# antgroup/ant-ray

Measured on NVIDIA H100. Metric: resnet50_ddp_train_images_per_sec, higher is better.
Workload: dtype bf16

## Files before the change

### ant-ray_b200/csrc/inst_norm.cu

```cuda
#include <algorithm>

#include "norm_kernels.cuh"
#include "norm_launch.h"

namespace b200c {
namespace bn {

static int ceil_div(int a, int b) { return (a + b - 1) / b; }

static int last_pow2(unsigned n) {
  n |= (n >> 1);
  n |= (n >> 2);
  n |= (n >> 4);
  n |= (n >> 8);
  n |= (n >> 16);
  return std::max<int>(1, n - (n >> 1));
}

static void reduce_config(int reduction, int stride, dim3* block, dim3* grid) {
  int block_x = std::min(last_pow2(stride), kTileW);
  int block_y = std::min(last_pow2(ceil_div(reduction, kElemsPerThread)), kMaxBlock / block_x);
  if (block_x * block_y != kMaxBlock) block_x = std::min(last_pow2(stride), kMaxBlock / block_y);
  int grid_y = std::min(ceil_div(reduction, block_y * kElemsPerThread), kMaxHBlock);
  *block = dim3(block_x, block_y, 1);
  *grid = dim3(ceil_div(stride, block_x), grid_y < 8 ? 1 : grid_y, 1);
}

static_assert(kEwVec % kStatsVec == 0, "vec_ok covers the statistics kernel's vector width");
static bool vec_ok(int stride, const void* const* ptrs, int n) {
  if (stride % kEwVec) return false;
  for (int i = 0; i < n; i++)
    if (reinterpret_cast<uintptr_t>(ptrs[i]) % 16) return false;
  return true;
}

static void ew_config(int reduction, int stride, int vec, dim3* block, dim3* grid) {
  const int groups = stride / vec;
  const int bx = std::min(groups, kEwThreads);
  const int by = kEwThreads / bx;
  const int gx = ceil_div(groups, bx);
  const int gy = std::max(1, std::min(ceil_div(reduction, by), 4096 / gx));
  *block = dim3(bx, by, 1);
  *grid = dim3(gx, gy, 1);
}

constexpr int kSemaphores = kMaxChannels / kTileW;
constexpr size_t kSemaphoreBytes = (size_t)kSemaphores * 4;

size_t scratch_bytes(int stride) {
  return kSemaphoreBytes + (size_t)3 * stride * kMaxHBlock * 4 + (size_t)2 * stride * 4;
}

struct Scratch {
  int* semaphores;
  float* staging;
  float* sums;
};
static Scratch carve(void* scratch, int stride) {
  char* p = static_cast<char*>(scratch);
  Scratch s;
  s.semaphores = reinterpret_cast<int*>(p);
  s.staging = reinterpret_cast<float*>(p + kSemaphoreBytes);
  s.sums = s.staging + (size_t)3 * stride * kMaxHBlock;
  return s;
}

cudaError_t forward(const FwdArgs& a, cudaStream_t st) {
  Scratch s = carve(a.scratch, a.c);
  dim3 block, grid;
  reduce_config(a.m, a.c, &block, &grid);
  StatsOut o{a.save_mean, a.save_invstd, a.running_mean, a.running_var, a.num_batches_tracked, a.momentum,
             (float)((double)a.m / (double)(a.m - 1)), a.eps};
  const bf16* x = static_cast<const bf16*>(a.x);
  if (vec_ok(a.c, &a.x, 1)) {
    k_bn_stats<kStatsVec><<<grid, dim3(block.x / kStatsVec, block.y), 0, st>>>(x, o, s.staging, s.semaphores, a.m, a.c);
  } else {
    k_bn_stats<1><<<grid, block, 0, st>>>(x, o, s.staging, s.semaphores, a.m, a.c);
  }
  const void* ptrs[3] = {a.x, a.y, a.identity ? a.identity : a.x};
  const int vec = vec_ok(a.c, ptrs, 3) ? kEwVec : 1;
  ew_config(a.m, a.c, vec, &block, &grid);
  const bf16* id = static_cast<const bf16*>(a.identity);
  bf16* y = static_cast<bf16*>(a.y);
#define B200C_BN_TRANSFORM(V, R) k_bn_transform<V, R><<<grid, block, 0, st>>>(x, id, y, a.save_mean, a.save_invstd, a.weight, a.bias, a.m, a.c)
  if (vec == kEwVec) {
    if (id) B200C_BN_TRANSFORM(kEwVec, true); else B200C_BN_TRANSFORM(kEwVec, false);
  } else {
    if (id) B200C_BN_TRANSFORM(1, true); else B200C_BN_TRANSFORM(1, false);
  }
#undef B200C_BN_TRANSFORM
  return cudaGetLastError();
}

cudaError_t backward(const BwdArgs& a, cudaStream_t st) {
  Scratch s = carve(a.scratch, a.c);
  float* sum_dy = s.sums;
  float* sum_dy_xmu = s.sums + a.c;
  dim3 block, grid;
  reduce_config(a.m, a.c, &block, &grid);
  const bf16* x = static_cast<const bf16*>(a.x);
  const bf16* dy = static_cast<const bf16*>(a.dy);
  const bf16* y = static_cast<const bf16*>(a.y);
  bf16* masked = static_cast<bf16*>(a.dy_masked);
  k_bn_bwd_reduce<<<grid, block, 0, st>>>(x, dy, y, masked, a.save_mean, a.save_invstd, sum_dy, sum_dy_xmu, a.grad_weight,
                                          a.grad_bias, s.staging, s.semaphores, a.m, a.c);
  const void* ptrs[4] = {a.x, a.dy, a.y, a.dx};
  const void* mptrs[3] = {a.x, a.dy_masked, a.dx};
  const int vec = (masked ? vec_ok(a.c, mptrs, 3) : vec_ok(a.c, ptrs, 4)) ? kEwVec : 1;
  ew_config(a.m, a.c, vec, &block, &grid);
  const float norm_fct = (float)(1.0 / a.m);
  bf16* dx = static_cast<bf16*>(a.dx);
#define B200C_BN_ELEMT(V, M, G) \
  k_bn_bwd_elemt<V, M><<<grid, block, 0, st>>>(G, y, x, dx, a.save_mean, a.save_invstd, a.weight, sum_dy, sum_dy_xmu, norm_fct, a.m, a.c)
  if (vec == kEwVec) {
    if (masked) B200C_BN_ELEMT(kEwVec, true, masked); else B200C_BN_ELEMT(kEwVec, false, dy);
  } else {
    if (masked) B200C_BN_ELEMT(1, true, masked); else B200C_BN_ELEMT(1, false, dy);
  }
#undef B200C_BN_ELEMT
  return cudaGetLastError();
}

}
}
```

### ant-ray_b200/csrc/norm_kernels.cuh

```cuda
#pragma once
#include <cuda_bf16.h>
#include <cuda_runtime.h>
#include <stdint.h>

namespace b200c {
namespace bn {

constexpr int kMaxBlock = 512;
constexpr int kParallelLoads = 4;
constexpr int kElemsPerThread = 16;
constexpr int kTileW = 32;
constexpr int kMaxHBlock = 128;
constexpr int kStatsVec = 4;
constexpr int kEwThreads = 256;
constexpr int kEwVec = 8;

typedef __nv_bfloat16 bf16;

template <int V>
struct alignas(2 * V) BVec {
  bf16 v[V];
};


template <bool FUSE_NEW>
__device__ __forceinline__ void welford_merge_element(int& count, float& mean, float& m2n, const int& count_new,
                                                      const float& mean_new, const float& m2n_new) {
  float factor = float(1.0) / ::max(1, (count + count_new));
  float delta0 = mean - mean_new;
  const float c = count, c_new = count_new;
  mean = __fmul_rn(FUSE_NEW ? __fmaf_rn(mean_new, c_new, __fmul_rn(mean, c)) : __fmaf_rn(mean, c, __fmul_rn(mean_new, c_new)),
                   factor);
  m2n = __fadd_rn(m2n, __fmaf_rn(__fmul_rn(__fmul_rn(__fmul_rn(delta0, delta0), c_new), c), factor, m2n_new));
  count += count_new;
}

template <int V>
__device__ __forceinline__ void welford_merge_block_vertical(int (&count)[V], float (&mean)[V], float (&m2n)[V],
                                                             int* shmem_count, float* shmem_mean, float* shmem_m2n) {
  const int block_x = blockDim.x * V;
  auto address_base = threadIdx.x * V + threadIdx.y * block_x;
#pragma unroll
  for (int offset = blockDim.y / 2; offset > 0; offset >>= 1) {
    if (threadIdx.y < offset * 2) {
#pragma unroll
      for (int k = 0; k < V; k++) {
        shmem_mean[address_base + k] = mean[k];
        shmem_m2n[address_base + k] = m2n[k];
        shmem_count[address_base + k] = count[k];
      }
    }
    __syncthreads();
    if (threadIdx.y < offset && threadIdx.y + offset < blockDim.y) {
      auto address = address_base + offset * block_x;
#pragma unroll
      for (int k = 0; k < V; k++) {
        auto count_new = shmem_count[address + k];
        auto mean_new = shmem_mean[address + k];
        auto m2n_new = shmem_m2n[address + k];
        welford_merge_element<false>(count[k], mean[k], m2n[k], count_new, mean_new, m2n_new);
      }
    }
  }
}

__device__ __forceinline__ void merge_block_vertical_backward(float& sum_dy, float& sum_dy_xmu, float* shmem_sum_dy,
                                                              float* shmem_sum_dy_xmu) {
  auto address_base = threadIdx.x + threadIdx.y * blockDim.x;
#pragma unroll
  for (int offset = blockDim.y / 2; offset > 0; offset >>= 1) {
    if (threadIdx.y < offset * 2) {
      shmem_sum_dy[address_base] = sum_dy;
      shmem_sum_dy_xmu[address_base] = sum_dy_xmu;
    }
    __syncthreads();
    if (threadIdx.y < offset && threadIdx.y + offset < blockDim.y) {
      auto address = address_base + offset * blockDim.x;
      sum_dy += shmem_sum_dy[address];
      sum_dy_xmu += shmem_sum_dy_xmu[address];
    }
  }
}

struct StatsOut {
  float* save_mean;
  float* save_invstd;
  float* running_mean;
  float* running_var;
  long long* num_batches_tracked;
  float momentum, bessel, eps;
};

__device__ __forceinline__ void finish_stats(const StatsOut& o, int c, float mean_th, float m2_th, int count_th) {
  const float mean = mean_th;
  const float var = m2_th / count_th;
  const float momentum = o.momentum;
  const float unbiased_var = var * o.bessel;
  o.save_mean[c] = mean;
  o.running_mean[c] = __fmaf_rn(mean, momentum, __fmul_rn(1 - momentum, o.running_mean[c]));
  o.running_var[c] = __fmaf_rn(unbiased_var, momentum, __fmul_rn(1 - momentum, o.running_var[c]));
  o.save_invstd[c] = rsqrtf(var + o.eps);
}

template <int V>
__global__ void __launch_bounds__(kMaxBlock / V) k_bn_stats(const bf16* __restrict__ input, StatsOut o, volatile float* staging_data,
                                                            int* semaphores, const int reduction_size, const int stride) {
  constexpr int PARALLEL_LOADS = kParallelLoads;
  float x_mean[PARALLEL_LOADS][V];
  float m_2_n[PARALLEL_LOADS][V];
  int count[PARALLEL_LOADS];
#pragma unroll
  for (int i = 0; i < PARALLEL_LOADS; i++) {
#pragma unroll
    for (int k = 0; k < V; k++) {
      x_mean[i][k] = 0.f;
      m_2_n[i][k] = 0.f;
    }
    count[i] = 0;
  }
  if (o.num_batches_tracked && blockIdx.x == 0 && blockIdx.y == 0 && threadIdx.x == 0 && threadIdx.y == 0)
    *o.num_batches_tracked += 1;

  int inner_loop_stride = blockDim.y * gridDim.y;
  int m_offset = blockIdx.y * blockDim.y + threadIdx.y;
  int c_offset = (blockIdx.x * blockDim.x + threadIdx.x) * V;
  int loop_count = 1 + (reduction_size - 1) / (inner_loop_stride * PARALLEL_LOADS);
  const bool c_valid = c_offset < stride;

  for (int i = 0; i < loop_count; i++) {
    BVec<V> xv[PARALLEL_LOADS];
#pragma unroll
    for (int j = 0; j < PARALLEL_LOADS; j++) {
      const int m = m_offset + j * inner_loop_stride;
      if (c_valid && m < reduction_size) xv[j] = *reinterpret_cast<const BVec<V>*>(input + ((size_t)m * stride + c_offset));
    }
#pragma unroll
    for (int j = 0; j < PARALLEL_LOADS; j++) {
      float x_math[V];
      float x_count_inv;
      float is_valid;
      if (c_valid && m_offset < reduction_size) {
#pragma unroll
        for (int k = 0; k < V; k++) x_math[k] = __bfloat162float(xv[j].v[k]);
        count[j]++;
        x_count_inv = float(1) / count[j];
        is_valid = float(1);
      } else {
#pragma unroll
        for (int k = 0; k < V; k++) x_math[k] = float(0);
        x_count_inv = float(0);
        is_valid = float(0);
      }
      m_offset += inner_loop_stride;
#pragma unroll
      for (int k = 0; k < V; k++) {
        float delta0 = x_math[k] - x_mean[j][k];
        x_mean[j][k] = __fmaf_rn(delta0, x_count_inv, x_mean[j][k]);
        float delta1 = x_math[k] - x_mean[j][k];
        m_2_n[j][k] = __fmaf_rn(__fmul_rn(delta0, delta1), is_valid, m_2_n[j][k]);
      }
    }
  }
  float mean_th[V], m2_th[V];
  int count_th[V];
#pragma unroll
  for (int k = 0; k < V; k++) {
    count_th[k] = count[0];
    mean_th[k] = x_mean[0][k];
    m2_th[k] = m_2_n[0][k];
#pragma unroll
    for (int j = 1; j < PARALLEL_LOADS; j++) welford_merge_element<true>(count_th[k], mean_th[k], m2_th[k], count[j], x_mean[j][k], m_2_n[j][k]);
  }

  __shared__ float shmem_mean[kMaxBlock];
  __shared__ float shmem_m2n[kMaxBlock];
  __shared__ int shmem_count[kMaxBlock];
  welford_merge_block_vertical<V>(count_th, mean_th, m2_th, shmem_count, shmem_mean, shmem_m2n);

  if (gridDim.y > 1) {
    volatile float* staging_mean = staging_data;
    volatile float* staging_m2n = &staging_data[stride * gridDim.y];
    volatile int* staging_count = reinterpret_cast<volatile int*>(&staging_m2n[stride * gridDim.y]);
    int address_base = c_offset + blockIdx.y * stride;
    if (threadIdx.y == 0 && c_valid) {
#pragma unroll
      for (int k = 0; k < V; k++) {
        staging_mean[address_base + k] = mean_th[k];
        staging_m2n[address_base + k] = m2_th[k];
        staging_count[address_base + k] = count_th[k];
      }
    }
    __threadfence();
    __syncthreads();
    __shared__ bool is_last_block_done;
    if (threadIdx.x == 0 && threadIdx.y == 0) {
      int old = atomicAdd(&semaphores[blockIdx.x], 1);
      is_last_block_done = (old == (gridDim.y - 1));
      if (is_last_block_done) semaphores[blockIdx.x] = 0;
    }
    __syncthreads();
    if (is_last_block_done) {
#pragma unroll
      for (int k = 0; k < V; k++) {
        count_th[k] = 0;
        mean_th[k] = float(0.0);
        m2_th[k] = float(0.0);
      }
      for (int y = threadIdx.y; y < gridDim.y; y += blockDim.y) {
        address_base = c_offset + y * stride;
#pragma unroll
        for (int k = 0; k < V; k++) {
          int count_new = c_valid ? staging_count[address_base + k] : 0;
          float mean_new = c_valid ? staging_mean[address_base + k] : float(0.0);
          float m2n_new = c_valid ? staging_m2n[address_base + k] : float(0.0);
          welford_merge_element<false>(count_th[k], mean_th[k], m2_th[k], count_new, mean_new, m2n_new);
        }
      }
      welford_merge_block_vertical<V>(count_th, mean_th, m2_th, shmem_count, shmem_mean, shmem_m2n);
      if (threadIdx.y == 0 && c_valid)
#pragma unroll
        for (int k = 0; k < V; k++) finish_stats(o, c_offset + k, mean_th[k], m2_th[k], count_th[k]);
    }
  } else {
    if (blockIdx.y == 0 && threadIdx.y == 0 && c_valid)
#pragma unroll
      for (int k = 0; k < V; k++) finish_stats(o, c_offset + k, mean_th[k], m2_th[k], count_th[k]);
  }
}

template <int V, bool RESID>
__global__ void __launch_bounds__(kEwThreads) k_bn_transform(const bf16* __restrict__ input, const bf16* __restrict__ identity,
                                                             bf16* __restrict__ out, const float* __restrict__ mean,
                                                             const float* __restrict__ inv_std, const float* __restrict__ weight,
                                                             const float* __restrict__ shift, const int reduction_size,
                                                             const int stride) {
  const int c0 = (blockIdx.x * blockDim.x + threadIdx.x) * V;
  if (c0 >= stride) return;
  float m_c[V], inv_std_c[V], w_c[V], s_c[V];
#pragma unroll
  for (int j = 0; j < V; j++) {
    m_c[j] = mean[c0 + j];
    inv_std_c[j] = inv_std[c0 + j];
    w_c[j] = weight[c0 + j];
    s_c[j] = shift[c0 + j];
  }
  const int row_step = blockDim.y * gridDim.y;
  for (int m = blockIdx.y * blockDim.y + threadIdx.y; m < reduction_size; m += row_step) {
    const int a = m * stride + c0;
    const BVec<V> xv = *reinterpret_cast<const BVec<V>*>(input + a);
    BVec<V> zv;
    if (RESID) zv = *reinterpret_cast<const BVec<V>*>(identity + a);
    BVec<V> yv;
#pragma unroll
    for (int j = 0; j < V; j++) {
      auto tmp = w_c[j] * (__bfloat162float(xv.v[j]) - m_c[j]) * inv_std_c[j] + s_c[j];
      if (RESID) {
        const bf16 r = __float2bfloat16(__bfloat162float(__float2bfloat16(tmp)) + __bfloat162float(zv.v[j]));
        yv.v[j] = __bfloat162float(r) <= 0.f ? __float2bfloat16(0.f) : r;
      } else {
        yv.v[j] = tmp <= 0.f ? __float2bfloat16(0.f) : __float2bfloat16(tmp);
      }
    }
    *reinterpret_cast<BVec<V>*>(out + a) = yv;
  }
}

__device__ __forceinline__ bf16 relu_grad(bf16 dy, bf16 y) { return __bfloat162float(y) <= 0.f ? __float2bfloat16(0.f) : dy; }

__global__ void k_bn_bwd_reduce(const bf16* __restrict__ input, const bf16* __restrict__ grad_output, const bf16* __restrict__ output,
                                bf16* __restrict__ masked, const float* __restrict__ mean, const float* __restrict__ inv_std,
                                float* __restrict__ sum_dy_o, float* __restrict__ sum_dy_xmu_o, float* __restrict__ grad_weight,
                                float* __restrict__ grad_bias, volatile float* staging_data, int* semaphores,
                                const int reduction_size, const int stride) {
  constexpr int PARALLEL_LOADS = kParallelLoads;
  float sum_dy[PARALLEL_LOADS];
  float sum_dy_xmu[PARALLEL_LOADS];
#pragma unroll
  for (int i = 0; i < PARALLEL_LOADS; i++) {
    sum_dy[i] = float(0);
    sum_dy_xmu[i] = float(0);
  }
  int inner_loop_stride = blockDim.y * gridDim.y;
  int m_offset = blockIdx.y * blockDim.y + threadIdx.y;
  int c_offset = blockIdx.x * blockDim.x + threadIdx.x;
  if (c_offset >= stride || m_offset >= reduction_size) return;

  int loop_count = 1 + (reduction_size - 1) / (inner_loop_stride * PARALLEL_LOADS);
  int address_base = m_offset * stride + c_offset;
  int address_increment = inner_loop_stride * stride;
  auto r_mean = mean[c_offset];
  auto factor = inv_std[c_offset];

  for (int i = 0; i < loop_count; i++) {
    bf16 dy_v[PARALLEL_LOADS], y_v[PARALLEL_LOADS], x_v[PARALLEL_LOADS];
#pragma unroll
    for (int j = 0; j < PARALLEL_LOADS; j++) {
      if (m_offset + j * inner_loop_stride < reduction_size) {
        const int a = address_base + j * address_increment;
        dy_v[j] = grad_output[a];
        y_v[j] = output[a];
        x_v[j] = input[a];
      }
    }
    float x_input[PARALLEL_LOADS];
    float x_grad_output[PARALLEL_LOADS];
#pragma unroll
    for (int j = 0; j < PARALLEL_LOADS; j++) {
      if (c_offset < stride && m_offset < reduction_size) {
        const bf16 g = relu_grad(dy_v[j], y_v[j]);
        if (masked) masked[address_base] = g;
        x_input[j] = __bfloat162float(x_v[j]);
        x_grad_output[j] = __bfloat162float(g);
      } else {
        x_input[j] = float(0);
        x_grad_output[j] = float(0);
      }
      m_offset += inner_loop_stride;
      address_base += address_increment;
    }
#pragma unroll
    for (int j = 0; j < PARALLEL_LOADS; j++) {
      sum_dy[j] += x_grad_output[j];
      sum_dy_xmu[j] = __fmaf_rn(x_grad_output[j], x_input[j] - r_mean, sum_dy_xmu[j]);
    }
  }
#pragma unroll
  for (int j = 1; j < PARALLEL_LOADS; j++) {
    sum_dy[0] += sum_dy[j];
    sum_dy_xmu[0] += sum_dy_xmu[j];
  }
  auto sum_dy_th = sum_dy[0];
  auto sum_dy_xmu_th = sum_dy_xmu[0];

  __shared__ float shmem_sum_dy[kMaxBlock];
  __shared__ float shmem_sum_dy_xmu[kMaxBlock];
  merge_block_vertical_backward(sum_dy_th, sum_dy_xmu_th, shmem_sum_dy, shmem_sum_dy_xmu);

  if (gridDim.y > 1) {
    volatile float* staging_sum_dy = staging_data;
    volatile float* staging_sum_dy_xmu = &staging_data[stride * gridDim.y];
    address_base = c_offset + blockIdx.y * stride;
    if (threadIdx.y == 0 && c_offset < stride) {
      staging_sum_dy[address_base] = sum_dy_th;
      staging_sum_dy_xmu[address_base] = sum_dy_xmu_th;
    }
    __threadfence();
    __syncthreads();
    __shared__ bool is_last_block_done;
    if (threadIdx.x == 0 && threadIdx.y == 0) {
      int old = atomicAdd(&semaphores[blockIdx.x], 1);
      is_last_block_done = (old == (gridDim.y - 1));
      if (is_last_block_done) semaphores[blockIdx.x] = 0;
    }
    __syncthreads();
    if (is_last_block_done) {
      sum_dy_th = float(0.0);
      sum_dy_xmu_th = float(0.0);
      for (int y = threadIdx.y; y < gridDim.y; y += blockDim.y) {
        address_base = c_offset + y * stride;
        sum_dy_th += (c_offset < stride ? staging_sum_dy[address_base] : float(0.0));
        sum_dy_xmu_th += (c_offset < stride ? staging_sum_dy_xmu[address_base] : float(0.0));
      }
      merge_block_vertical_backward(sum_dy_th, sum_dy_xmu_th, shmem_sum_dy, shmem_sum_dy_xmu);
      if (threadIdx.y == 0 && c_offset < stride) {
        grad_bias[c_offset] = sum_dy_th;
        grad_weight[c_offset] = sum_dy_xmu_th * factor;
        sum_dy_o[c_offset] = sum_dy_th;
        sum_dy_xmu_o[c_offset] = sum_dy_xmu_th;
      }
    }
  } else {
    if (blockIdx.y == 0 && threadIdx.y == 0 && c_offset < stride) {
      grad_bias[c_offset] = sum_dy_th;
      grad_weight[c_offset] = sum_dy_xmu_th * factor;
      sum_dy_o[c_offset] = sum_dy_th;
      sum_dy_xmu_o[c_offset] = sum_dy_xmu_th;
    }
  }
}

template <int V, bool MASKED>
__global__ void __launch_bounds__(kEwThreads) k_bn_bwd_elemt(const bf16* __restrict__ grad_output, const bf16* __restrict__ output,
                                                             const bf16* __restrict__ input, bf16* __restrict__ grad_input,
                                                             const float* __restrict__ mean, const float* __restrict__ inv_std,
                                                             const float* __restrict__ weight, const float* __restrict__ sum_dy,
                                                             const float* __restrict__ sum_dy_xmu, const float norm_fct,
                                                             const int reduction_size, const int stride) {
  const int c0 = (blockIdx.x * blockDim.x + threadIdx.x) * V;
  if (c0 >= stride) return;
  float m_c[V], m_dy_c[V], factor_1_c[V], factor_2_c[V];
#pragma unroll
  for (int j = 0; j < V; j++) {
    m_c[j] = mean[c0 + j];
    m_dy_c[j] = sum_dy[c0 + j] * norm_fct;
    factor_1_c[j] = inv_std[c0 + j];
    factor_2_c[j] = weight[c0 + j] * factor_1_c[j];
    factor_1_c[j] = factor_1_c[j] * factor_1_c[j] * sum_dy_xmu[c0 + j] * norm_fct;
  }
  const int row_step = blockDim.y * gridDim.y;
  for (int m = blockIdx.y * blockDim.y + threadIdx.y; m < reduction_size; m += row_step) {
    const int a = m * stride + c0;
    const BVec<V> gv = *reinterpret_cast<const BVec<V>*>(grad_output + a);
    BVec<V> yv;
    if (!MASKED) yv = *reinterpret_cast<const BVec<V>*>(output + a);
    const BVec<V> xv = *reinterpret_cast<const BVec<V>*>(input + a);
    BVec<V> dxv;
#pragma unroll
    for (int j = 0; j < V; j++) {
      const float g = __bfloat162float(MASKED ? gv.v[j] : relu_grad(gv.v[j], yv.v[j]));
      dxv.v[j] = __float2bfloat16((g - m_dy_c[j] - (__bfloat162float(xv.v[j]) - m_c[j]) * factor_1_c[j]) * factor_2_c[j]);
    }
    *reinterpret_cast<BVec<V>*>(grad_input + a) = dxv;
  }
}

}
}
```

Baseline: 4766.

## Pipeline BN stats and backward-reduce loads through cp.async shared-memory rings

The batch-norm statistics kernel now streams its vectorized input loads through a four-stage cp.async ring in shared memory and gets a min-blocks-per-SM launch bound. The backward reduce kernel, when pointers are 16-byte aligned, has warps cooperatively issue 16-byte cp.async copies of dy, y and x into a two-stage ring before each thread reads back its own scalar elements. The aim is to hide global-memory latency in these bandwidth-bound reductions by overlapping loads with compute. In exchange it adds shared-memory footprint and per-warp index bookkeeping, and the backward ring keeps inactive threads alive to take part in copies.

Result: faster. 4843 (median of 6 runs) (+1.6%).

```diff
diff --git a/ant-ray_b200/csrc/inst_norm.cu b/ant-ray_b200/csrc/inst_norm.cu
--- a/ant-ray_b200/csrc/inst_norm.cu
+++ b/ant-ray_b200/csrc/inst_norm.cu
@@ -102,8 +102,12 @@
   const bf16* dy = static_cast<const bf16*>(a.dy);
   const bf16* y = static_cast<const bf16*>(a.y);
   bf16* masked = static_cast<bf16*>(a.dy_masked);
-  k_bn_bwd_reduce<<<grid, block, 0, st>>>(x, dy, y, masked, a.save_mean, a.save_invstd, sum_dy, sum_dy_xmu, a.grad_weight,
-                                          a.grad_bias, s.staging, s.semaphores, a.m, a.c);
+  const void* rptrs[3] = {a.x, a.dy, a.y};
+#define B200C_BN_BWD_REDUCE(RING)                                                                                  \
+  k_bn_bwd_reduce<RING><<<grid, block, 0, st>>>(x, dy, y, masked, a.save_mean, a.save_invstd, sum_dy, sum_dy_xmu, \
+                                                a.grad_weight, a.grad_bias, s.staging, s.semaphores, a.m, a.c)
+  if (vec_ok(a.c, rptrs, 3)) B200C_BN_BWD_REDUCE(true); else B200C_BN_BWD_REDUCE(false);
+#undef B200C_BN_BWD_REDUCE
   const void* ptrs[4] = {a.x, a.dy, a.y, a.dx};
   const void* mptrs[3] = {a.x, a.dy_masked, a.dx};
   const int vec = (masked ? vec_ok(a.c, mptrs, 3) : vec_ok(a.c, ptrs, 4)) ? kEwVec : 1;
diff --git a/ant-ray_b200/csrc/norm_kernels.cuh b/ant-ray_b200/csrc/norm_kernels.cuh
--- a/ant-ray_b200/csrc/norm_kernels.cuh
+++ b/ant-ray_b200/csrc/norm_kernels.cuh
@@ -12,6 +12,9 @@
 constexpr int kTileW = 32;
 constexpr int kMaxHBlock = 128;
 constexpr int kStatsVec = 4;
+constexpr int kStatsStages = 4;
+constexpr int kStatsBlocksPerSm = 8;
+constexpr int kBwdStages = 2;
 constexpr int kEwThreads = 256;
 constexpr int kEwVec = 8;
 
@@ -21,6 +24,18 @@
 struct alignas(2 * V) BVec {
   bf16 v[V];
 };
+
+template <int BYTES>
+__device__ __forceinline__ void cp_async_zfill(void* dst, const void* src, bool valid) {
+  const unsigned d = static_cast<unsigned>(__cvta_generic_to_shared(dst));
+  if constexpr (BYTES == 16)
+    asm volatile("cp.async.cg.shared.global [%0], [%1], 16, %2;\n" ::"r"(d), "l"(src), "r"(valid ? 16 : 0) : "memory");
+  else
+    asm volatile("cp.async.ca.shared.global [%0], [%1], %2, %3;\n" ::"r"(d), "l"(src), "n"(BYTES), "r"(valid ? BYTES : 0) : "memory");
+}
+__device__ __forceinline__ void cp_async_commit() { asm volatile("cp.async.commit_group;\n" ::: "memory"); }
+template <int N>
+__device__ __forceinline__ void cp_async_wait() { asm volatile("cp.async.wait_group %0;\n" ::"n"(N) : "memory"); }
 
 
 template <bool FUSE_NEW>
@@ -103,7 +118,7 @@
 }
 
 template <int V>
-__global__ void __launch_bounds__(kMaxBlock / V) k_bn_stats(const bf16* __restrict__ input, StatsOut o, volatile float* staging_data,
+__global__ void __launch_bounds__(kMaxBlock / V, V == kStatsVec ? kStatsBlocksPerSm : 0) k_bn_stats(const bf16* __restrict__ input, StatsOut o, volatile float* staging_data,
                                                             int* semaphores, const int reduction_size, const int stride) {
   constexpr int PARALLEL_LOADS = kParallelLoads;
   float x_mean[PARALLEL_LOADS][V];
@@ -127,38 +142,71 @@
   int loop_count = 1 + (reduction_size - 1) / (inner_loop_stride * PARALLEL_LOADS);
   const bool c_valid = c_offset < stride;
 
-  for (int i = 0; i < loop_count; i++) {
-    BVec<V> xv[PARALLEL_LOADS];
-#pragma unroll
-    for (int j = 0; j < PARALLEL_LOADS; j++) {
-      const int m = m_offset + j * inner_loop_stride;
-      if (c_valid && m < reduction_size) xv[j] = *reinterpret_cast<const BVec<V>*>(input + ((size_t)m * stride + c_offset));
-    }
-#pragma unroll
-    for (int j = 0; j < PARALLEL_LOADS; j++) {
-      float x_math[V];
-      float x_count_inv;
-      float is_valid;
-      if (c_valid && m_offset < reduction_size) {
-#pragma unroll
-        for (int k = 0; k < V; k++) x_math[k] = __bfloat162float(xv[j].v[k]);
-        count[j]++;
-        x_count_inv = float(1) / count[j];
-        is_valid = float(1);
-      } else {
-#pragma unroll
-        for (int k = 0; k < V; k++) x_math[k] = float(0);
-        x_count_inv = float(0);
-        is_valid = float(0);
-      }
-      m_offset += inner_loop_stride;
-#pragma unroll
-      for (int k = 0; k < V; k++) {
-        float delta0 = x_math[k] - x_mean[j][k];
-        x_mean[j][k] = __fmaf_rn(delta0, x_count_inv, x_mean[j][k]);
-        float delta1 = x_math[k] - x_mean[j][k];
-        m_2_n[j][k] = __fmaf_rn(__fmul_rn(delta0, delta1), is_valid, m_2_n[j][k]);
-      }
+  auto update = [&](const int j, const BVec<V>& xv) {
+    float x_math[V];
+    float x_count_inv;
+    float is_valid;
+    if (c_valid && m_offset < reduction_size) {
+#pragma unroll
+      for (int k = 0; k < V; k++) x_math[k] = __bfloat162float(xv.v[k]);
+      count[j]++;
+      x_count_inv = float(1) / count[j];
+      is_valid = float(1);
+    } else {
+#pragma unroll
+      for (int k = 0; k < V; k++) x_math[k] = float(0);
+      x_count_inv = float(0);
+      is_valid = float(0);
+    }
+    m_offset += inner_loop_stride;
+#pragma unroll
+    for (int k = 0; k < V; k++) {
+      float delta0 = x_math[k] - x_mean[j][k];
+      x_mean[j][k] = __fmaf_rn(delta0, x_count_inv, x_mean[j][k]);
+      float delta1 = x_math[k] - x_mean[j][k];
+      m_2_n[j][k] = __fmaf_rn(__fmul_rn(delta0, delta1), is_valid, m_2_n[j][k]);
+    }
+  };
+  if constexpr (V == kStatsVec) {
+    constexpr int S = kStatsStages;
+    __shared__ alignas(16) BVec<V> ring[S][PARALLEL_LOADS][kMaxBlock / V];
+    const int tid = threadIdx.x + threadIdx.y * blockDim.x;
+    const int m_first = m_offset;
+    const size_t row_step = (size_t)inner_loop_stride * stride;
+    auto issue = [&](int it) {
+      if (it < loop_count) {
+        const int m0 = m_first + it * PARALLEL_LOADS * inner_loop_stride;
+        const bf16* src = input + ((size_t)m0 * stride + c_offset);
+#pragma unroll
+        for (int j = 0; j < PARALLEL_LOADS; j++) {
+          const bool ok = c_valid && m0 + j * inner_loop_stride < reduction_size;
+          cp_async_zfill<sizeof(BVec<V>)>(&ring[it % S][j][tid], ok ? src + j * row_step : input, ok);
+        }
+      }
+      cp_async_commit();
+    };
+#pragma unroll
+    for (int s = 0; s < S - 1; s++) issue(s);
+    for (int i = 0; i < loop_count; i++) {
+      issue(i + S - 1);
+      cp_async_wait<S - 1>();
+#pragma unroll
+      for (int j = 0; j < PARALLEL_LOADS; j += 2) {
+        const BVec<V> x0 = ring[i % S][j][tid], x1 = ring[i % S][j + 1][tid];
+        update(j, x0);
+        update(j + 1, x1);
+      }
+    }
+  } else {
+    for (int i = 0; i < loop_count; i++) {
+      BVec<V> xv[PARALLEL_LOADS];
+#pragma unroll
+      for (int j = 0; j < PARALLEL_LOADS; j++) {
+        const int m = m_offset + j * inner_loop_stride;
+        if (c_valid && m < reduction_size) xv[j] = *reinterpret_cast<const BVec<V>*>(input + ((size_t)m * stride + c_offset));
+      }
+#pragma unroll
+      for (int j = 0; j < PARALLEL_LOADS; j++) update(j, xv[j]);
     }
   }
   float mean_th[V], m2_th[V];
@@ -267,6 +315,7 @@
 
 __device__ __forceinline__ bf16 relu_grad(bf16 dy, bf16 y) { return __bfloat162float(y) <= 0.f ? __float2bfloat16(0.f) : dy; }
 
+template <bool RING>
 __global__ void k_bn_bwd_reduce(const bf16* __restrict__ input, const bf16* __restrict__ grad_output, const bf16* __restrict__ output,
                                 bf16* __restrict__ masked, const float* __restrict__ mean, const float* __restrict__ inv_std,
                                 float* __restrict__ sum_dy_o, float* __restrict__ sum_dy_xmu_o, float* __restrict__ grad_weight,
@@ -283,25 +332,16 @@
   int inner_loop_stride = blockDim.y * gridDim.y;
   int m_offset = blockIdx.y * blockDim.y + threadIdx.y;
   int c_offset = blockIdx.x * blockDim.x + threadIdx.x;
-  if (c_offset >= stride || m_offset >= reduction_size) return;
+  const bool active = c_offset < stride && m_offset < reduction_size;
+  if (!RING && !active) return;
 
   int loop_count = 1 + (reduction_size - 1) / (inner_loop_stride * PARALLEL_LOADS);
   int address_base = m_offset * stride + c_offset;
   int address_increment = inner_loop_stride * stride;
-  auto r_mean = mean[c_offset];
-  auto factor = inv_std[c_offset];
-
-  for (int i = 0; i < loop_count; i++) {
-    bf16 dy_v[PARALLEL_LOADS], y_v[PARALLEL_LOADS], x_v[PARALLEL_LOADS];
-#pragma unroll
-    for (int j = 0; j < PARALLEL_LOADS; j++) {
-      if (m_offset + j * inner_loop_stride < reduction_size) {
-        const int a = address_base + j * address_increment;
-        dy_v[j] = grad_output[a];
-        y_v[j] = output[a];
-        x_v[j] = input[a];
-      }
-    }
+  auto r_mean = mean[active ? c_offset : 0];
+  auto factor = inv_std[active ? c_offset : 0];
+
+  auto accumulate = [&](const bf16(&dy_v)[PARALLEL_LOADS], const bf16(&y_v)[PARALLEL_LOADS], const bf16(&x_v)[PARALLEL_LOADS]) {
     float x_input[PARALLEL_LOADS];
     float x_grad_output[PARALLEL_LOADS];
 #pragma unroll
@@ -322,6 +362,74 @@
     for (int j = 0; j < PARALLEL_LOADS; j++) {
       sum_dy[j] += x_grad_output[j];
       sum_dy_xmu[j] = __fmaf_rn(x_grad_output[j], x_input[j] - r_mean, sum_dy_xmu[j]);
+    }
+  };
+  if constexpr (RING) {
+    constexpr int S = kBwdStages;
+    constexpr int kOps = 3;
+    __shared__ alignas(16) bf16 ring[S][PARALLEL_LOADS][kOps][kMaxBlock];
+    const int tid = threadIdx.x + threadIdx.y * blockDim.x;
+    const int lane = tid & 31, warp0 = tid & ~31;
+    const int lanes = min(32, (int)(blockDim.x * blockDim.y) - warp0);
+    const unsigned warp_mask = lanes == 32 ? 0xffffffffu : (1u << lanes) - 1;
+    const int groups = lanes / 8;
+    const bool second = lane < lanes / 2;
+    const bf16* chunk_src[2];
+    int chunk_m[2], chunk_dst[2];
+    bool chunk_c_ok[2];
+#pragma unroll
+    for (int k = 0; k < 2; k++) {
+      const int q = lane + k * lanes;
+      const int j = q / groups / kOps, op = q / groups % kOps;
+      const int t0 = warp0 + 8 * (q % groups);
+      const int c = blockIdx.x * blockDim.x + t0 % blockDim.x;
+      chunk_c_ok[k] = c < stride;
+      chunk_src[k] = (op == 0 ? grad_output : op == 1 ? output : input) + c;
+      chunk_m[k] = blockIdx.y * blockDim.y + t0 / blockDim.x + j * inner_loop_stride;
+      chunk_dst[k] = (j * kOps + op) * kMaxBlock + t0;
+    }
+    auto issue = [&](int it) {
+      if (it < loop_count) {
+#pragma unroll
+        for (int k = 0; k < 2; k++) {
+          if (k == 0 || second) {
+            const int m = chunk_m[k] + it * PARALLEL_LOADS * inner_loop_stride;
+            const bool ok = chunk_c_ok[k] && m < reduction_size;
+            cp_async_zfill<16>(&ring[it % S][0][0][0] + chunk_dst[k], ok ? chunk_src[k] + (size_t)m * stride : grad_output, ok);
+          }
+        }
+      }
+      cp_async_commit();
+    };
+#pragma unroll
+    for (int s = 0; s < S - 1; s++) issue(s);
+    for (int i = 0; i < loop_count; i++) {
+      cp_async_wait<S - 2>();
+      __syncwarp(warp_mask);
+      issue(i + S - 1);
+      bf16 dy_v[PARALLEL_LOADS], y_v[PARALLEL_LOADS], x_v[PARALLEL_LOADS];
+#pragma unroll
+      for (int j = 0; j < PARALLEL_LOADS; j++) {
+        dy_v[j] = ring[i % S][j][0][tid];
+        y_v[j] = ring[i % S][j][1][tid];
+        x_v[j] = ring[i % S][j][2][tid];
+      }
+      accumulate(dy_v, y_v, x_v);
+    }
+    if (!active) return;
+  } else {
+    for (int i = 0; i < loop_count; i++) {
+      bf16 dy_v[PARALLEL_LOADS], y_v[PARALLEL_LOADS], x_v[PARALLEL_LOADS];
+#pragma unroll
+      for (int j = 0; j < PARALLEL_LOADS; j++) {
+        if (m_offset + j * inner_loop_stride < reduction_size) {
+          const int a = address_base + j * address_increment;
+          dy_v[j] = grad_output[a];
+          y_v[j] = output[a];
+          x_v[j] = input[a];
+        }
+      }
+      accumulate(dy_v, y_v, x_v);
     }
   }
 #pragma unroll
```
